# shiv-vignesh/T5-Resnet-VQA

Hardware: AMD Instinct MI355X
Metric: question-image pairs/sec, ResNet50+T5-base+SGA train step, 1/2/4/8 MI355X (higher is better)
Workload: dtype bf16; 1 GPU; ResNet50 + t5-base + 3xSGA train step (BASELINE configs[1]; configs[2] at N=8); model=resnet50+t5-base+3xSGA, global_batch=64, per_gpu_batch=64, seq_len=32, image_size=224, answers=170, parallelism=dp1, world_size=1, graph=True, resnet_pipelined=True

## Files before the change

include/vqa_hip.h:

```cpp
#ifndef VQA_HIP_H
#define VQA_HIP_H

#include <hip/hip_runtime.h>

#ifdef __cplusplus
extern "C" {
#endif

#define VQA_ABI_VERSION 22
#define VQA_OK 0
#define VQA_ERR_INVALID 1000

int vqa_abi_version(void);
const char* vqa_last_error(void);

typedef struct vqa_dropout {
  float p;
  unsigned site;
  const unsigned* rng;
} vqa_dropout;

int vqa_rng_advance(unsigned* rng, hipStream_t stream);
int vqa_dropout_mask(const vqa_dropout* d, float* out, long long n, hipStream_t stream);

// ... 232 lines not shown

int vqa_eval_rows(const vqa_eval_desc* d, hipStream_t stream);

#define VQA_MAX_GROUPS 8
#define VQA_ST_STEP 0
#define VQA_ST_GRAD_NORM 1
#define VQA_ST_CLIP_COEF 2
#define VQA_ST_LR_SCALE 3
#define VQA_ST_BC1 4
#define VQA_ST_BC2_SQRT 5
#define VQA_ST_PENDING 8

typedef struct vqa_adamw_desc {
  float* param; const float* grad;
  float* exp_avg; float* exp_avg_sq; float* max_exp_avg_sq;
  void* param16;
  long long n;
  int ngroups;
  long long group_end[VQA_MAX_GROUPS];
  float group_lr[VQA_MAX_GROUPS];
  float beta1, beta2, eps, weight_decay, grad_scale;
  const float* state;
} vqa_adamw_desc;

int vqa_grad_sqnorm(const float* g, long long n, double* ws, int parts, hipStream_t stream);
int vqa_optim_finalize(const double* ws, int parts, float grad_scale, float max_norm, int warmup, int total,
                       float beta1, float beta2, float* state, hipStream_t stream);
#define VQA_SQNORM_FINAL_COUNTER_WORDS 2112
int vqa_grad_sqnorm_final(const float* g0, long long n0, const float* g1, long long n1, double* ws, int parts,
                          int fin_parts, const int* mark, long long lead, int cols, unsigned* counter,
                          float grad_scale, float max_norm, int warmup, int total, float beta1, float beta2,
                          float* state, hipStream_t stream);
int vqa_adamw_amsgrad(const vqa_adamw_desc* d, hipStream_t stream);
int vqa_embed_mark(const long long* ids, int n, int rows, int* mark, const float* state, hipStream_t stream);
int vqa_adamw_rows(const vqa_adamw_desc* d, const int* mark, int rows, int cols, int touched, int warmup, int total,
                   hipStream_t stream);

#ifdef __cplusplus
}
#endif
#endif
```

t5-resnet-vqa_amd/csrc/adamw.h:

```cpp
#pragma once
#include "common.h"

namespace {

struct AdamArgs {
  float* p; const float* g; float* m; float* v; float* vm; bf16_t* p16;
  long n4;
  int ngroups; long gend4[VQA_MAX_GROUPS]; float glr[VQA_MAX_GROUPS];
  float b1, b2, eps, wd, gscale;
  const float* st;
};

inline int adam_args(const vqa_adamw_desc* d, AdamArgs& A) {
  VQA_REQUIRE(d && d->param && d->grad && d->exp_avg && d->exp_avg_sq && d->max_exp_avg_sq && d->state,
              "vqa_adamw: null argument");
  VQA_REQUIRE(d->n > 0 && d->n % 4 == 0 && d->ngroups >= 1 && d->ngroups <= VQA_MAX_GROUPS, "vqa_adamw: bad sizes");
  VQA_REQUIRE((((uintptr_t)d->param | (uintptr_t)d->grad | (uintptr_t)d->exp_avg | (uintptr_t)d->exp_avg_sq |
                (uintptr_t)d->max_exp_avg_sq) & 15) == 0 && ((uintptr_t)d->param16 & 7) == 0,
              "vqa_adamw: the fp32 streams must be 16-byte aligned, param16 8-byte aligned");
  A.p = d->param; A.g = d->grad; A.m = d->exp_avg; A.v = d->exp_avg_sq; A.vm = d->max_exp_avg_sq;
  A.p16 = (bf16_t*)d->param16;
  A.n4 = d->n / 4;
  A.ngroups = d->ngroups;
  for (int i = 0; i < VQA_MAX_GROUPS; ++i) {
    VQA_REQUIRE(i >= d->ngroups || d->group_end[i] % 4 == 0, "vqa_adamw: group ends must be multiples of 4");
    A.gend4[i] = i < d->ngroups ? d->group_end[i] / 4 : A.n4;
    A.glr[i] = i < d->ngroups ? d->group_lr[i] : 0.f;
  }
  A.b1 = d->beta1; A.b2 = d->beta2; A.eps = d->eps; A.wd = d->weight_decay; A.gscale = d->grad_scale;
  A.st = d->state;
  return VQA_OK;
}

__device__ __forceinline__ void adamw_update4_with(const AdamArgs& A, long i, f32x4_t& p, const f32x4_t g4,
                                                   f32x4_t& m, f32x4_t& v, f32x4_t& vm, const float coef,
                                                   const float lam, const float bc1, const float bc2s) {
#pragma clang fp contract(off)
  const float gmul = A.gscale * coef;
  const float omb1 = 1.f - A.b1, omb2 = 1.f - A.b2;
  int gi = 0;
#pragma unroll
  for (int k = 0; k < VQA_MAX_GROUPS - 1; ++k) gi += (k < A.ngroups - 1 && i >= A.gend4[k]) ? 1 : 0;
  const float lr = A.glr[gi] * lam;
  const float decay = 1.f - lr * A.wd, step_size = lr / bc1;
#pragma unroll
  for (int j = 0; j < 4; ++j) {
    const float gr = g4[j] * gmul;
    p[j] *= decay;
    m[j] = m[j] + omb1 * (gr - m[j]);
    v[j] = v[j] * A.b2 + omb2 * gr * gr;
    vm[j] = fmaxf(vm[j], v[j]);
    const float denom = sqrtf(vm[j]) / bc2s + A.eps;
    p[j] = p[j] - step_size * (m[j] / denom);
  }
}

__device__ __forceinline__ void adamw_update4(const AdamArgs& A, long i, f32x4_t& p, const f32x4_t g4, f32x4_t& m,
                                              f32x4_t& v, f32x4_t& vm) {
  adamw_update4_with(A, i, p, g4, m, v, vm, A.st[VQA_ST_CLIP_COEF], A.st[VQA_ST_LR_SCALE], A.st[VQA_ST_BC1],
                     A.st[VQA_ST_BC2_SQRT]);
}

}
```

t5-resnet-vqa_amd/csrc/optim.hip:

```cpp
#include "adamw.h"

namespace {

__device__ __forceinline__ double sq_term(const float4 v) {
  return (double)v.x * v.x + (double)v.y * v.y + (double)v.z * v.z + (double)v.w * v.w;
}

__device__ __forceinline__ double sq_range(const float* __restrict__ g, long n4, int bid, int nblk) {
  const float4* g4 = reinterpret_cast<const float4*>(g);
  const long st = (long)nblk * 256;
  double s = 0.0;
  long i = (long)bid * 256 + threadIdx.x;
  for (; i + 3 * st < n4; i += 4 * st) {
    float4 v[4];
#pragma unroll
    for (int u = 0; u < 4; ++u) v[u] = g4[i + u * st];
#pragma unroll
    for (int u = 0; u < 4; ++u) s += sq_term(v[u]);
  }
  for (; i < n4; i += st) s += sq_term(g4[i]);
  return s;
}

__device__ __forceinline__ double sq_range_rows(const float* __restrict__ g, long n4, int bid, int nblk,
// ... 118 lines not shown
  s = sq_block_sum(s, red);
  int* flag = reinterpret_cast<int*>(red + 8);
  if (threadIdx.x == 0) {
    __hip_atomic_store((gu64*)(A.ws + (A.fin - 2 * K) + b), (unsigned long long)__double_as_longlong(s),
                       __ATOMIC_RELAXED, __HIP_MEMORY_SCOPE_AGENT);
    asm volatile("s_waitcnt vmcnt(0)" ::: "memory");
    const int nb = 2 * K, grp = b % SQ_NSUB;
    const unsigned members = (unsigned)((nb - grp + SQ_NSUB - 1) / SQ_NSUB);
    const unsigned groups = (unsigned)(nb < SQ_NSUB ? nb : SQ_NSUB);
    gu32* sub = (gu32*)(A.cnt + (1 + grp) * SQ_CNT_STRIDE);
    int last = 0;
    if (__hip_atomic_fetch_add(sub, 1u, __ATOMIC_RELAXED, __HIP_MEMORY_SCOPE_AGENT) == members - 1) {
      __hip_atomic_store(sub, 0u, __ATOMIC_RELAXED, __HIP_MEMORY_SCOPE_AGENT);
      last = __hip_atomic_fetch_add((gu32*)A.cnt, 1u, __ATOMIC_RELAXED, __HIP_MEMORY_SCOPE_AGENT) == groups - 1;
      if (last) __hip_atomic_store((gu32*)A.cnt, 0u, __ATOMIC_RELAXED, __HIP_MEMORY_SCOPE_AGENT);
    }
    *flag = last;
  }
  __syncthreads();
  if (!*flag) return;
  __syncthreads();
  __builtin_amdgcn_fence(__ATOMIC_ACQUIRE, "wavefront");
  finalize_body<true>(A.ws, A.fin, A.grad_scale, A.max_norm, A.warmup, A.total, A.beta1, A.beta2, A.st, red);
}

__global__ __launch_bounds__(256) void embed_mark_kernel(const long long* __restrict__ ids, int n, int rows,
                                                         int* __restrict__ mark, const float* __restrict__ st) {
  const int i = blockIdx.x * 256 + threadIdx.x;
  if (i >= n) return;
  const long long id = ids[i];
  if (id >= 0 && id < rows) mark[id] = (int)st[VQA_ST_STEP];
}

template <int MODE>
__global__ __launch_bounds__(192) void adamw_rows_kernel(AdamArgs A, const int* __restrict__ mark, int rows, int d4,
                                                         int warmup, int total) {
  const int step = (int)A.st[VQA_ST_STEP];
  float coef, lam, bc1, bc2s;
  if (MODE == 0) {
    coef = 1.f;
    schedule_at((double)A.st[VQA_ST_STEP], warmup, total, A.b1, A.b2, lam, bc1, bc2s);
  } else {
    if (A.st[VQA_ST_PENDING] == 0.f) return;
    coef = A.st[VQA_ST_CLIP_COEF];
    lam = A.st[VQA_ST_LR_SCALE];
    bc1 = A.st[VQA_ST_BC1];
    bc2s = A.st[VQA_ST_BC2_SQRT];
  }
  for (int row = blockIdx.x; row < rows; row += gridDim.x) {
  const bool touched = mark[row] == (MODE == 0 ? step : step - 1);
  if (MODE == 0 ? touched : !touched) continue;
  for (int c = threadIdx.x; c < d4; c += 192) {
    const long i = (long)row * d4 + c;
    f32x4_t p = __builtin_nontemporal_load(reinterpret_cast<const f32x4_t*>(A.p) + i);
    f32x4_t g4 = {0.f, 0.f, 0.f, 0.f};
    if (MODE == 1) g4 = __builtin_nontemporal_load(reinterpret_cast<const f32x4_t*>(A.g) + i);
    f32x4_t m = __builtin_nontemporal_load(reinterpret_cast<const f32x4_t*>(A.m) + i);
    f32x4_t v = __builtin_nontemporal_load(reinterpret_cast<const f32x4_t*>(A.v) + i);
    f32x4_t vm = __builtin_nontemporal_load(reinterpret_cast<const f32x4_t*>(A.vm) + i);
    adamw_update4_with(A, i, p, g4, m, v, vm, coef, lam, bc1, bc2s);
    __builtin_nontemporal_store(p, reinterpret_cast<f32x4_t*>(A.p) + i);
    __builtin_nontemporal_store(m, reinterpret_cast<f32x4_t*>(A.m) + i);
    __builtin_nontemporal_store(v, reinterpret_cast<f32x4_t*>(A.v) + i);
    __builtin_nontemporal_store(vm, reinterpret_cast<f32x4_t*>(A.vm) + i);
    if (A.p16) {
      uint2 u;
      u.x = (uint32_t)f2bf(p[0]) | ((uint32_t)f2bf(p[1]) << 16);
      u.y = (uint32_t)f2bf(p[2]) | ((uint32_t)f2bf(p[3]) << 16);
      reinterpret_cast<uint2*>(A.p16)[i] = u;
    }
  }
  }
}

__global__ __launch_bounds__(256) void adamw_kernel(AdamArgs A) {
  const long i = (long)blockIdx.x * 256 + threadIdx.x;
  if (i >= A.n4 || A.st[VQA_ST_PENDING] == 0.f) return;
  f32x4_t p = __builtin_nontemporal_load(reinterpret_cast<const f32x4_t*>(A.p) + i);
  const f32x4_t g4 = __builtin_nontemporal_load(reinterpret_cast<const f32x4_t*>(A.g) + i);
  f32x4_t m = __builtin_nontemporal_load(reinterpret_cast<const f32x4_t*>(A.m) + i);
  f32x4_t v = __builtin_nontemporal_load(reinterpret_cast<const f32x4_t*>(A.v) + i);
  f32x4_t vm = __builtin_nontemporal_load(reinterpret_cast<const f32x4_t*>(A.vm) + i);
  adamw_update4(A, i, p, g4, m, v, vm);
  __builtin_nontemporal_store(p, reinterpret_cast<f32x4_t*>(A.p) + i);
  __builtin_nontemporal_store(m, reinterpret_cast<f32x4_t*>(A.m) + i);
  __builtin_nontemporal_store(v, reinterpret_cast<f32x4_t*>(A.v) + i);
  __builtin_nontemporal_store(vm, reinterpret_cast<f32x4_t*>(A.vm) + i);
  if (A.p16) {
    uint2 u;
    u.x = (uint32_t)f2bf(p[0]) | ((uint32_t)f2bf(p[1]) << 16);
    u.y = (uint32_t)f2bf(p[2]) | ((uint32_t)f2bf(p[3]) << 16);
    reinterpret_cast<uint2*>(A.p16)[i] = u;
  }
}

int grid_for(long n4) {
  long b = (n4 + 255) / 256;
  return (int)(b < 4096 ? b : 4096);
}

}

extern "C" int vqa_grad_sqnorm(const float* g, long long n, double* ws, int parts, hipStream_t s) {
  VQA_REQUIRE(g && ws && n % 4 == 0 && parts > 0 && ((uintptr_t)g & 15) == 0,
              "vqa_grad_sqnorm: bad arguments (n %% 4 == 0, g 16-byte aligned)");
  hipLaunchKernelGGL(sqnorm_kernel, dim3(parts), dim3(256), 0, s, g, (long)(n / 4), ws);
  return vqa::check_launch("vqa_grad_sqnorm");
// ... 18 lines not shown
                        (n1 - lead) % cols == 0 && n1 / 4 < (1ll << 31)),
              "vqa_grad_sqnorm_final: range 1 must be `lead` floats then whole rows of `cols` (both %% 4 == 0)");
  SqFinalArgs A;
  A.g0 = g0; A.n4_0 = (long)(n0 / 4); A.g1 = g1; A.n4_1 = (long)(n1 / 4);
  A.ws = ws; A.parts = parts; A.fin = fin_parts;
  A.mark = mark; A.lead4 = (long)(lead / 4); A.d4 = mark ? (unsigned)(cols / 4) : 1u;
  A.cnt = counter;
  A.grad_scale = grad_scale; A.max_norm = max_norm; A.warmup = warmup; A.total = total;
  A.beta1 = beta1; A.beta2 = beta2; A.st = state;
  hipLaunchKernelGGL(sqnorm_final_kernel, dim3(2 * parts), dim3(256), 0, s, A);
  return vqa::check_launch("vqa_grad_sqnorm_final");
}

extern "C" int vqa_adamw_amsgrad(const vqa_adamw_desc* d, hipStream_t s) {
  AdamArgs A;
  if (int rc = adam_args(d, A)) return rc;
  hipLaunchKernelGGL(adamw_kernel, dim3(vqa::cdiv(A.n4, 256)), dim3(256), 0, s, A);
  return vqa::check_launch("vqa_adamw_amsgrad");
}

extern "C" int vqa_embed_mark(const long long* ids, int n, int rows, int* mark, const float* state, hipStream_t s) {
  VQA_REQUIRE(ids && mark && state && n > 0 && rows > 0, "vqa_embed_mark: bad arguments");
  hipLaunchKernelGGL(embed_mark_kernel, dim3(vqa::cdiv(n, 256)), dim3(256), 0, s, ids, n, rows, mark, state);
  return vqa::check_launch("vqa_embed_mark");
}

extern "C" int vqa_adamw_rows(const vqa_adamw_desc* d, const int* mark, int rows, int cols, int touched, int warmup,
                              int total, hipStream_t s) {
  AdamArgs A;
  if (int rc = adam_args(d, A)) return rc;
  VQA_REQUIRE(mark && rows > 0 && cols > 0 && cols % 4 == 0 && (long long)rows * cols == d->n,
              "vqa_adamw_rows: rows x cols must be the descriptor's n (cols %% 4 == 0)");
  const int grid = touched > 1 && touched < rows ? touched : rows;
  if (touched == 1)
    hipLaunchKernelGGL(adamw_rows_kernel<1>, dim3(rows), dim3(192), 0, s, A, mark, rows, cols / 4, warmup, total);
  else
    hipLaunchKernelGGL(adamw_rows_kernel<0>, dim3(grid), dim3(192), 0, s, A, mark, rows, cols / 4, warmup, total);
  return vqa::check_launch("vqa_adamw_rows");
}
```

t5-resnet-vqa_amd/dp.py:

```python
from __future__ import annotations

import os

import numpy as np
import torch

from . import lib as L
from . import ops
from . import synthetic as S
from .engine_base import _after, no_gc_capture


DP_T5_DW_GROUPS = (4, 4, 3, 1)


def dp_t5_dw_groups(layers=12):
    if layers == 12:
        return DP_T5_DW_GROUPS
    g = [layers // 3, layers // 3, layers // 4]
    return tuple(g + [layers - sum(g)])


def plan_buckets(ready_marks, end, min_bytes=24 << 20):
    out, start = [], 0
# ... 251 lines not shown
            full, mine = e.G32[a:a + N * c], e.G32[a + r * c:a + (r + 1) * c]
            if _staged(full, self.group) or dist.get_backend(self.group) == "gloo":
                h = full.cpu()
                dist.all_reduce(h, group=self.group)
                mine.copy_(h[r * c:(r + 1) * c])
                works.append(_Done())
            else:
                out = self.RS_OUT[self.rs_off[bk_index]:self.rs_off[bk_index] + c]
                if COMM_ON_STREAM:
                    dist.reduce_scatter_tensor(out, full, group=self.group, async_op=False)
                    mine.copy_(out)
                    works.append(_OnStream())
                else:
                    works.append(_Then(dist.reduce_scatter_tensor(out, full, group=self.group, async_op=True),
                                       lambda out=out, mine=mine: mine.copy_(out)))
        if b > a + N * c:
            works += allreduce_buckets(e.G32, [(None, a + N * c, b)], self.group)
        return [_All(works)]

    def _sharded_optimizer(self):
        import torch.distributed as dist
        e = self.eng
        s = L.stream_handle()
        self.WS_SQN.zero_()
        for c in self.sq_calls:
            c(s)
        if _staged(self.WS_SQN, self.group):
            h = self.WS_SQN.cpu()
            dist.all_reduce(h, group=self.group)
            self.WS_SQN.copy_(h)
        else:
            dist.all_reduce(self.WS_SQN, group=self.group)
        self.finalize_call(s)
        for c in self.adam_calls:
            c(s)
        e.clear_pending(s)
        N, r = self.world, self.rank
        for a, c, b in self.shards:
            if c == 0:
                continue
            for t in (e.P32, e.P16):
                full, mine = t[a:a + N * c], t[a + r * c:a + (r + 1) * c]
                if _staged(full, self.group):
                    parts = [torch.empty(c, dtype=t.dtype) for _ in range(N)]
                    dist.all_gather(parts, mine.cpu(), group=self.group)
                    full.copy_(torch.cat(parts))
                else:
                    dist.all_gather_into_tensor(full, mine.clone(), group=self.group)
        if e.fp8 and not e.defer_opt:
            self._run(e.quant_all)

    def sync_optimizer_state(self):
        import torch.distributed as dist
        if not self.shard:
            return
        e = self.eng
        N, r = self.world, self.rank
        for a, c, b in self.shards:
            if c == 0:
                continue
            for t in (e.M, e.V, e.VMAX):
                full, mine = t[a:a + N * c], t[a + r * c:a + (r + 1) * c]
                if _staged(full, self.group):
                    parts = [torch.empty(c, dtype=t.dtype) for _ in range(N)]
                    dist.all_gather(parts, mine.cpu(), group=self.group)
                    full.copy_(torch.cat(parts))
# ... 93 lines not shown
                    for k in st["final"]:
                        works[k] = exchange(k, self.buckets[k])
                        mark_done(k, works[k])
                else:
                    ks = st["final"]
                    assert ks == list(range(ks[0], ks[-1] + 1))
                    ws = allreduce_buckets(e.G32, [(None, self.buckets[ks[0]][1], self.buckets[ks[-1]][2])], self.group)
                    for k in ks:
                        works[k] = ws if k == ks[-1] else []
                        mark_done(k, ws)
                    if j == self._sq0_stage and (COMM_ON_STREAM or _staged(e.G32, self.group)):
                        self._sq0_call(L.stream_handle(comm))
        if tm is not None:
            tm["wait"] = (torch.cuda.Event(enable_timing=True), torch.cuda.Event(enable_timing=True))
            tm["wait"][0].record(main)
        for key, ws in works.items():
            for w in ws:
                w.wait()
        _after(main, comm)
        if tm is not None:
            tm["wait"][1].record(main)
        self._play("finish", self.finish_calls)
        return tm

    def _play(self, name, calls):
        if self.graphs is not None:
            self.graphs[name].replay()
        else:
            self._run(calls)

    def capture(self):
        e = self.eng
        e.flush_optimizer()
        e.ROWTOT.fill_(float(e.B * self.world))
        s = torch.cuda.Stream(e.dev)
        s.wait_stream(torch.cuda.current_stream(e.dev))
        saved_rng = e.RNG.clone()
        with torch.cuda.stream(s):
            e._run(e.fwd_calls)
            e.backward()
        torch.cuda.current_stream(e.dev).wait_stream(s)
        torch.cuda.synchronize(e.dev)
        e.RNG.copy_(saved_rng)
        with no_gc_capture():
            self.graphs = self._capture_all(s)

    def _capture_all(self, s):
        e = self.eng
        gs = {}

        def cap(name, fn):
            g = torch.cuda.CUDAGraph()
            with torch.cuda.graph(g, stream=s):
                fn()
            gs[name] = g
        cap("fwd", self._fwd)
        for j, st in enumerate(self.stages):
            cap(f"stage{j}", lambda st=st: self._run_stage(st))
        cap("finish", lambda: self._run(self.finish_calls))
        return gs

    def _fwd(self):
        e = self.eng
        main = torch.cuda.current_stream(e.dev)
        if self._res_a:
            _after(e._rstream, main)
            with torch.cuda.stream(e._rstream):
                self._run(self._res_a)
        e.run_forward_streams()
        if self._res_a:
            _after(main, e._rstream)

    def _exchange_step_start(self):
        e = self.eng
        main = torch.cuda.current_stream(e.dev)
        e.count_call(L.stream_handle(main))
        _after(self._comm, main)
        with torch.cuda.stream(self._comm):
            ws = allreduce_buckets(e.ROWTOT, [(None, 0, 1)], self.group)
            return ws + gather_tensor(e.IDS, self.GIDS, self.group)

    def step(self):
        e = self.eng
        rows = self._exchange_step_start()
        if e.pipeline:
            e.copy_f4(L.stream_handle(torch.cuda.current_stream(e.dev)))
        if self.graphs is not None:
            self.graphs["fwd"].replay()
        else:
            self._fwd()
        for w in rows:
            w.wait()
        _after(torch.cuda.current_stream(e.dev), self._comm)
        tev = self._backward_exchange()
        if self.shard:
            self._sharded_optimizer()
        if self.timing:
            self._ev.append(tev)

    def timing_report(self):
        torch.cuda.synchronize()
        if not self._ev:
            return None
        e = self.eng
        stage_of = {k: j for j, st in enumerate(self.stages) for k in st["final"]}
        stage_of["rows"] = self.rows_stage

        def mean(f):
            return round(float(np.mean([f(t) for t in self._ev])), 1)
        lag = {k: mean(lambda t, k=k: t["stage"][stage_of[k]].elapsed_time(t["done"][k]) * 1e3) for k in stage_of}
        return {"world_size": self.world, "steps": len(self._ev), "stages": self.stage_plan(),
                "embedding_rows_gather": {"bytes": int(self.world * e.T * (e.D * 4 + 8)),
                                          "done_us_after_stage": lag["rows"]},
                "buckets": [{"start": int(a), "stop": int(b), "bytes": int(4 * (b - a)), "stage": stage_of[k],
                             "done_us_after_stage": lag[k]} for k, (_, a, b) in enumerate(self.buckets)],
                "exposed_wait_us_total": mean(lambda t: t["wait"][0].elapsed_time(t["wait"][1]) * 1e3)}
# ... 1 lines not shown
```

t5-resnet-vqa_amd/engine.py:

```python
from __future__ import annotations

import ctypes
import os

import numpy as np
import torch

from . import lib as L
from . import ops
from . import synthetic as S
from .engine_base import (BF16, F32, I64, IGNORE_INDEX, SITE_EMBED, SITE_FINAL, EngineBase, _after,
                          _check_attn_path, _h2d, _Seq, batch_rows, load_rows, load_rows_multi, no_gc_capture,
                          t5_site)
from .layout import ParamLayout, fold_bn, t5_bucket_map
from .sga_stack import SGAGrads, SGAStack, sga_site
from .t5_stack import T5Grads, T5Stack


def stem_s2d_weight(wf):
    co, kh, kw, ci = wf.shape
    w8 = np.zeros((co, 8, 8, ci), np.float32)
    w8[:, :kh, :kw] = wf
    w = w8.reshape(co, 4, 2, 4, 2, ci).transpose(0, 1, 3, 2, 4, 5).reshape(co, 4, 4, 4 * ci)
    return np.concatenate([w, np.zeros((co, 4, 4, 16 - 4 * ci), np.float32)], 3)


class VQAEngine(EngineBase):
    def __init__(self, state_dict, vision="resnet50", batch=64, seq_len=32, image_size=224, device="cuda:0",
                 warmup=10, total=100, num_blocks=3, answer_spaces=170, grad_scale=1.0, max_norm=1.0,
                 betas=(0.9, 0.999), eps=1e-8, weight_decay=0.1, dropout=0.1, seed=0, pipeline=False,
                 t5_dw_group=None, defer_optimizer=True, dw_stream=None, sga_dw_batch=True, pair_bwd=True,
                 language_model="t5-base", fp8=False, sga_attn_group=True, fuse_norm=None):
        super().__init__(device, dropout, seed, warmup, total, max_norm, betas, eps, weight_decay, grad_scale)
        self.fuse_norm = (os.environ.get("VQA_FUSE_NORM", "0") == "1") if fuse_norm is None else bool(fuse_norm)
        self.fuse_norm_kept = []
        self.pipeline = bool(pipeline)
        self.res_order, self.res_head = "first", 4
        self._res_feed = None
        self._rstream_handle = None
        self._rstream_plain = None
        self.EMB_MARK = None
        self.SQ_CNT = None
        self.heat_call = None
        self._fpn_plan = None
        self.vision, self.B, self.L, self.H = vision, batch, seq_len, image_size
        assert image_size % 2 == 0, "the space-to-depth stem needs an even image size"
        self.NB, self.A = num_blocks, answer_spaces
        self.dims = dm = S.lm_dims(language_model)
        self.D, self.nl, self.h5, self.dkv, self.dff = dm.d_model, dm.t5_layers, dm.t5_heads, dm.t5_dkv, dm.t5_dff
        self.sga_heads, self.sga_dh = dm.sga_heads, dm.sga_dhead
        assert self.h5 * self.dkv == self.D and self.sga_heads * self.sga_dh == self.D
        self.fp8 = bool(fp8)
        if not 1 <= answer_spaces <= 1024:
            raise ValueError(f"answer_spaces={answer_spaces}: the fused answer head supports 1..1024 answers")
        if not 1 <= seq_len <= 64:
            raise ValueError(f"seq_len={seq_len}: the attention / pooler kernels support 1..64 question tokens")
        self.pair_bwd = bool(pair_bwd)
        if t5_dw_group is None:
            t5_dw_group = (3 * self.nl // 4, self.nl - 3 * self.nl // 4)
        if isinstance(t5_dw_group, (list, tuple)):
            self.t5_dw_groups = [int(x) for x in t5_dw_group]
        elif int(t5_dw_group) == 1:
            self.t5_dw_groups = None
        else:
            G = int(t5_dw_group)
            assert G > 1, "t5_dw_group: a group size >= 1 or a sequence of sizes"
            self.t5_dw_groups = [G] * (self.nl // G) + [self.nl % G] * (self.nl % G > 0)
        assert self.t5_dw_groups is None or (sum(self.t5_dw_groups) == self.nl and min(self.t5_dw_groups) >= 1)
        self.sga_dw_batch = bool(sga_dw_batch)
        self.sga_attn_group = bool(sga_attn_group)
        self.defer_opt = bool(defer_optimizer)
        self.dw_stream = True if dw_stream is None else bool(dw_stream)
        self.T = batch * seq_len
        self.rows = batch
# ... 406 lines not shown
            if quant[name]:
                c = _Seq([c] + quant[name])
            if name == "embed":
                self.adam_embed = c
            else:
                self.adam_segs.append((name, c))
        lst = []
        self._call(lst, "vqa_zero", ops.addr(self.opt_state, L.ST_PENDING), 16, extra=[self.opt_state])
        self.clear_pending = lst[0]
        if not self.defer_opt:
            o.append(self.adam_full)
            o += self.quant_all
        elif self.adam_embed is not None:
            o.append(self.adam_embed)
        self.embed_split = self.defer_opt
        self.tail_calls = o[2:]
        self.emb_pre = []
        if self.embed_split:
            emb = lay["t5.embed"]
            assert emb.offset + emb.numel == n and self.adam_embed is o[-1]
            if self.EMB_MARK is None:
                self.EMB_MARK = torch.full((S.T5_VOCAB,), -1, dtype=torch.int32, device=self.dev)
            lo = emb.offset
            self._emb_desc = dt = self._adam_range_desc(lo, n)
            keep = self._adam_keep() + (self.EMB_MARK,)
            rows_call = lambda touched: ops.Call("vqa_adamw_rows", ctypes.byref(dt), self.EMB_MARK.data_ptr(),
                                                 S.T5_VOCAB, self.D, touched, int(self.warmup), int(self.total),
                                                 desc=dt, keep=keep)
            self.emb_pre = [ops.Call("vqa_embed_mark", self.IDS.data_ptr(), self.T, S.T5_VOCAB,
                                     self.EMB_MARK.data_ptr(), self.opt_state.data_ptr(),
                                     keep=(self.IDS, self.EMB_MARK, self.opt_state)),
                            rows_call(256)]
            self.tail_calls = o[2:-1] + [self.adam_range_call(lay["t5.relbias"].offset, lo), rows_call(1)]
        self.tail_calls_unfused = self.tail_calls
        T = self.T
        self.fused_tail = self.embed_split and T <= 16384
        self.emb_sort_call = self.emb_scatter_call = None
        if self.fused_tail:
            if self.SQ_CNT is None:
                self.SQ_CNT = torch.zeros(L.SQNORM_FINAL_COUNTER_WORDS, dtype=torch.int32,
                                          device=self.dev)
            emb = lay["t5.embed"]
            lead = emb.offset - e0
            assert lead >= 0 and lead % 4 == 0 and emb.numel == S.T5_VOCAB * self.D and self.D % 4 == 0
            fin = ops.Call("vqa_grad_sqnorm_final", ops.addr(self.G32, a), e0 - a, ops.addr(self.G32, e0), n - e0,
                           self.WS_SQ.data_ptr(), K, 3 * K, self.EMB_MARK.data_ptr(), lead, self.D,
                           self.SQ_CNT.data_ptr(), float(self.grad_scale), float(self.max_norm), int(self.warmup),
                           int(self.total), float(self.betas[0]), float(self.betas[1]), self.opt_state.data_ptr(),
                           keep=(self.G32[a:], self.WS_SQ, self.EMB_MARK, self.SQ_CNT, self.opt_state))
            assert [c.name for c in self.tail_calls[:2]] == ["vqa_grad_sqnorm", "vqa_optim_finalize"]
            self.tail_calls = [fin] + self.tail_calls[2:]
            ids, dh, dtab, _, _, _, ws = self.emb_call.args
            self.emb_sort_call = ops.Call("vqa_embedding_sort", ids, T, S.T5_VOCAB, ws, keep=(self.IDS, self.WS_EMB))
            self.emb_scatter_call = ops.Call("vqa_embedding_bwd_sorted", dh, dtab, T, self.D, S.T5_VOCAB, ws,
                                             keep=(self.dH32, self.G32, self.WS_EMB))

    def _adam_groups(self):
        ends, lrs = self.lay.group_of_element()
        return ends, [self.group_lr.get(g, lr) for g, lr in zip(self.lay.groups, lrs)]

    def flush_optimizer(self):
        if self.defer_opt:
            self._run([c for _, c in self.adam_segs] + [self.clear_pending])

    def set_grad_scale(self, s):
        self.grad_scale = float(s)
# ... 29 lines not shown
    def prime(self, images):
        assert self.pipeline, "prime() is for pipelined engines"
        ni = batch_rows({"image_tensors": images}, "image_tensors", self.B, self.allow_empty_rows)
        load_rows(self.IMG, images, ni)
        self._img_rows_next = ni
        self._run(self.res_calls)

    def use_global_rows(self, world):
        i = next(k for k, c in enumerate(self.bwd_calls) if c.name == "vqa_head_bwd")
        old = self.bwd_calls[i]
        if self.count_call is not None:
            assert old.args[-1] == float(world), "use_global_rows: already set for another world size"
            return
        new = ops.Call("vqa_head_bwd", *old.args[:-2], ops.addr(self.ROWTOT), float(world),
                       keep=tuple(old.keep) + (self.ROWTOT,))
        new.side = old.side
        self.bwd_calls[i] = new
        self.count_call = ops.Call("vqa_count_targets", ops.addr(self.TGT), self.B, ops.addr(self.ROWTOT),
                                   keep=(self.TGT, self.ROWTOT))
        self.allow_empty_rows = True
        self.graph = None

    def forward(self):
        self.flush_optimizer()
        super().forward()

    def _run_step_streams(self, optimizer=True):
        self.run_forward_streams()
        if optimizer:
            self._backward_and_tail()
        else:
            self.run_backward_streams()

    def _backward_and_tail(self):
        self.run_backward_streams(sq_overlap=True, sorted_scatter=self.fused_tail)
        self._run(self.tail_calls)

    def run_forward_streams(self):
        main = torch.cuda.current_stream(self.dev)
        side = self._side
        f = self.fwd_calls
        p0, p1, p2 = self._fsplit
        self._run(f[:p0])
        _after(side, main)
        vis, txt = f[p0:p1], f[p1:p2]
        if self.defer_opt:
            self._forward_branches_deferred(main, side, vis, txt)
        else:
            self._forward_branches(main, side, vis, txt)
        self._run(f[p2:])

    def _forward_branches(self, main, side, vis, txt):
        hm, hs = L.stream_handle(main), L.stream_handle(side)
        j = 0
        for i, c in enumerate(vis):
            c(hm)
            upto = (i + 1) * len(txt) // len(vis)
            while j < upto:
                txt[j](hs)
                j += 1
        for c in txt[j:]:
            c(hs)
        _after(main, side)

    def _t5_waits(self, i):
        w = [f"t5.{i}"]
        if self.fuse_norm and i + 1 < self.nl:
# ... 160 lines not shown
            g.replay()
        with torch.cuda.stream(self._rstream):
            self._run(self.res_calls)
        _after(main, self._rstream)

    def _step_pipelined(self):
        main = torch.cuda.current_stream(self.dev)
        if self.res_external:
            self.run_forward_streams()
            self._backward_and_tail()
            return
        if not (torch.cuda.is_current_stream_capturing() and self.res_order == "root"):
            self.copy_f4(L.stream_handle(main))
        _after(self._rstream, main)

        last = self.res_order == "last"
        inter = self.res_order == "interleave"
        if inter:
            self._res_feed = [list(self.res_calls), L.stream_handle(self._rstream)]
        elif not last:
            with torch.cuda.stream(self._rstream):
                self._run(self.res_calls)
        self.run_forward_streams()
        if inter:
            assert not self._res_feed[0], "every ResNet call issued"
            self._res_feed = None
        self._backward_and_tail()
        if last:
            with torch.cuda.stream(self._rstream):
                self._run(self.res_calls)
        _after(main, self._rstream)

    def train_step(self):
        if self.graph is not None and self.res_external:
            self._res_external_step()
            return
        if self.graph is not None and self.pipeline and self.res_order == "root":
            self.copy_f4(L.stream_handle(torch.cuda.current_stream(self.dev)))
        if self.graph is not None:
            for g in self.graph:
                if callable(g):
                    g()
                else:
                    g.replay()
            return
        if self.pipeline:
            assert self.allreduce is None, "pipelined DP steps go through dp.DataParallelStep"
            self._step_pipelined()
            return
        self.forward()
        self.backward()
        if self.allreduce is not None:
            self.allreduce(self.G32)
        self.optimizer_step()

    def capture(self, warm=True, keep_graph=False):
        self._keep_graph = bool(keep_graph)
        self.flush_optimizer()
        s = torch.cuda.Stream(self.dev)
        s.wait_stream(torch.cuda.current_stream(self.dev))
        saved, saved_rng = self.opt_state.clone(), self.RNG.clone()
        with torch.cuda.stream(s):
            if warm:
                self._run(self.fwd_calls)
                self.backward()
        torch.cuda.current_stream(self.dev).wait_stream(s)
        torch.cuda.synchronize(self.dev)
        with no_gc_capture():
            parts = self._capture_parts(s)
        self.opt_state.copy_(saved)
        self.RNG.copy_(saved_rng)
        for g in parts:
            if self._keep_graph and not callable(g):
                g.instantiate()
        self.graph = parts

    def _capture_parts(self, s):
        if self.allreduce is None:
            g = self._new_graph()
            with torch.cuda.graph(g, stream=s):
                if self.pipeline:
                    self._step_pipelined()
                else:
                    self._run_step_streams()
            parts = [g]
        else:
            g1, g2 = self._new_graph(), self._new_graph()
            with torch.cuda.graph(g1, stream=s):
                self.forward()
                self.backward()
            with torch.cuda.graph(g2, stream=s):
                self.optimizer_step()
            ar = self.allreduce
            parts = [g1, lambda: ar(self.G32), g2]
        return parts

    def _eval_setup(self, rollout):
        if self.pipeline:
            raise ValueError("pipelined engines take their images a step early; evaluation has no next batch: "
                             "build the engine with pipeline=False to evaluate")
        super()._eval_setup(rollout)

    def _eval_heat_setup(self, heatmap):
        if heatmap:
            self._plan_heat()

    def _run_eval_streams(self):
        main = torch.cuda.current_stream(self.dev)
        side = self._side
        f = self.fwd_calls
# ... 67 lines not shown
```

t5-resnet-vqa_amd/lib.py:

```python
from __future__ import annotations

import ctypes
import os
import re

import torch

PKG_DIR = os.path.dirname(os.path.abspath(__file__))
LIB_PATH = os.path.join(PKG_DIR, "lib", "libvqa_hip.so")
HEADER = os.path.join(os.path.dirname(PKG_DIR), "include", "vqa_hip.h")

c_void_p, c_int, c_float, c_ll = ctypes.c_void_p, ctypes.c_int, ctypes.c_float, ctypes.c_longlong


class ConvGeom(ctypes.Structure):
    _fields_ = [(n, c_int) for n in ("n", "h", "w", "c", "oh", "ow", "kh", "kw", "stride", "pad")]


class Dropout(ctypes.Structure):
    _fields_ = [("p", c_float), ("site", ctypes.c_uint), ("rng", c_void_p)]


class GemmDesc(ctypes.Structure):
    _fields_ = [
# ... 67 lines not shown
                           f"{[int(r[0]) for r in rows]}")
    return {int(r[0]): tuple(map(int, r[1:7])) + (frozenset(re.findall(r"VQA_TILE_(\w+)", r[7])),) for r in rows}


def _flagged(flag):
    return tuple(c for c, t in _TILE_TABLE.items() if flag in t[6])


_TILE_TABLE = gemm_tile_table()
GEMM_TILES = {c: t[:3] for c, t in _TILE_TABLE.items()}
GEMM_WAVES = {c: t[3:5] for c, t in _TILE_TABLE.items()}
GEMM_PATCH_ONLY = _flagged("PATCH")
GEMM_KC_B_ONLY = _flagged("KC_B")
GEMM_K64_ONLY = _flagged("K1")
GEMM_FP8 = _flagged("FP8")
GEMM_NORM = _flagged("NORM")
GEMM_PAIR = _flagged("PAIR")
GEMM_BK128 = tuple(c for c, t in _TILE_TABLE.items() if t[5] == 128)
GEMM_PLAIN_ONLY = tuple(sorted(GEMM_BK128 + GEMM_K64_ONLY))
GEMM_NO_SPLITK = tuple(sorted(GEMM_PLAIN_ONLY + GEMM_PATCH_ONLY))
NORM_LAYER, NORM_RMS = 1, 2


def gemm_config_fits(cfg, d):
    im2col = bool(d.a_conv or d.b_conv)
    return not ((cfg in GEMM_PATCH_ONLY) != (d.a_conv == 2) or (d.norm and cfg not in GEMM_NORM)
                or (d.fp8 and cfg not in GEMM_FP8) or (cfg in GEMM_KC_B_ONLY and d.b_trans)
                or (cfg in GEMM_PLAIN_ONLY and im2col) or (cfg in GEMM_K64_ONLY and d.k > 64))

ATTN_MFMA, ATTN_LONG, ATTN_VALU = 0, 1, 2
MAX_GROUPS = 8
ST_STEP, ST_GRAD_NORM, ST_CLIP_COEF, ST_LR_SCALE, ST_BC1, ST_BC2_SQRT = range(6)
ST_PENDING, ST_FLOATS = 8, 16


class AdamWDesc(ctypes.Structure):
    _fields_ = [
        ("param", c_void_p), ("grad", c_void_p), ("exp_avg", c_void_p), ("exp_avg_sq", c_void_p),
        ("max_exp_avg_sq", c_void_p), ("param16", c_void_p), ("n", c_ll), ("ngroups", c_int),
        ("group_end", c_ll * MAX_GROUPS), ("group_lr", c_float * MAX_GROUPS),
        ("beta1", c_float), ("beta2", c_float), ("eps", c_float), ("weight_decay", c_float),
        ("grad_scale", c_float), ("state", c_void_p),
    ]


class EvalDesc(ctypes.Structure):
    _fields_ = [
        ("logp", c_void_p), ("targets", c_void_p), ("nll", c_void_p), ("loss", c_void_p), ("similarity", c_void_p),
        ("batch", c_int), ("answers", c_int), ("k", c_int),
        ("topk_idx", c_void_p), ("topk_logp", c_void_p), ("acc", c_void_p),
        ("pred_log", c_void_p), ("tgt_log", c_void_p), ("capacity", c_ll),
    ]


EVAL_MAX_K = 16
EVAL_ACC_INTS = ("steps", "rows", "top1", "topk", "cursor")
EVAL_ACC_F64 = ("loss_sum", "nll_sum", "sim_sum")

_lib = None


def header_symbols():
    txt = open(HEADER).read()
    return sorted(set(re.findall(r"^\s*(?:int|long long|const char\*)\s+(vqa_\w+)\s*\(", txt, re.M)))


def abi_version():
    return int(re.search(r"#define VQA_ABI_VERSION (\d+)", open(HEADER).read()).group(1))


def load():
    global _lib
    if _lib is not None:
        return _lib
    if not os.path.exists(LIB_PATH):
        raise RuntimeError(f"libvqa_hip.so not built at {LIB_PATH}: run `python __graft_entry__.py` "
                           "(make -C t5-resnet-vqa_amd/csrc)")
    lib = ctypes.CDLL(LIB_PATH)
    missing = [s for s in header_symbols() if not hasattr(lib, s)]
    if missing:
        raise RuntimeError(f"libvqa_hip.so lacks exported symbols {missing}")
    lib.vqa_last_error.restype = ctypes.c_char_p
    if lib.vqa_abi_version() != abi_version():
        raise RuntimeError(f"libvqa_hip.so ABI {lib.vqa_abi_version()} != header ABI {abi_version()}: rebuild it")
    lib.vqa_gemm.argtypes = [ctypes.POINTER(GemmDesc), c_void_p]
    lib.vqa_gemm_select.argtypes = [ctypes.POINTER(GemmDesc)]
    lib.vqa_gemm_workspace_bytes.argtypes = [ctypes.POINTER(GemmDesc)]
    lib.vqa_gemm_workspace_bytes.restype = c_ll
    lib.vqa_gemm_pair.argtypes = [ctypes.POINTER(GemmDesc), ctypes.POINTER(GemmDesc), c_void_p]
    lib.vqa_attn_fwd.argtypes = [ctypes.POINTER(AttnDesc), c_void_p]
    lib.vqa_attn_bwd.argtypes = [ctypes.POINTER(AttnDesc), c_void_p]
    lib.vqa_attn_path.argtypes = [ctypes.POINTER(AttnDesc), c_int]
    lib.vqa_attn_probs.argtypes = [ctypes.POINTER(AttnDesc), c_void_p]
    lib.vqa_attn_headmean.argtypes = [ctypes.POINTER(AttnDesc), c_void_p, c_ll, c_void_p]
    lib.vqa_adamw_amsgrad.argtypes = [ctypes.POINTER(AdamWDesc), c_void_p]
    lib.vqa_eval_rows.argtypes = [ctypes.POINTER(EvalDesc), c_void_p]
    lib.vqa_adamw_rows.argtypes = [ctypes.POINTER(AdamWDesc), c_void_p, c_int, c_int, c_int, c_int, c_int, c_void_p]
    for name in ("vqa_norm_bwd_workspace_floats", "vqa_colsum_workspace_floats"):
        getattr(lib, name).argtypes = [c_int, c_int]
    lib.vqa_head_workspace_floats.argtypes = [c_int] * 4
    lib.vqa_norm_bwd_parts.argtypes = [c_int]
    lib.vqa_colsum_parts.argtypes = [c_int]
    for name, argtypes in _SIGS.items():
        fn = getattr(lib, name)
        fn.argtypes = argtypes
        fn.restype = c_int
    _lib = lib
    return lib


_SIGS: dict = {}


def register(name, *argtypes):
    _SIGS[name] = list(argtypes) + [c_void_p]


P = c_void_p
register("vqa_rmsnorm_fwd", P, P, P, P, P, c_int, c_int, c_float, P)
register("vqa_rmsnorm_bwd", P, P, P, P, P, P, P, P, c_float, P, c_int, c_int, P, P, P)
register("vqa_layernorm_fwd", P, P, P, P, P, P, P, c_int, c_int, c_float)
register("vqa_layernorm_bwd", P, P, P, P, P, P, P, P, P, P, P, c_int, c_int, P, P)
register("vqa_rng_advance", P)
register("vqa_dropout_mask", P, P, c_ll)
register("vqa_colsum_partials", P, c_int, c_ll, c_int, P, c_float)
register("vqa_image_to_nhwc8", P, P, c_int, c_int, c_int)
register("vqa_image_to_s2d16", P, P, c_int, c_int, c_int)
register("vqa_resize_linear_u8", P, P, c_int, c_int, c_int, P)
register("vqa_resize_pil_bilinear_u8", P, P, c_int, c_int, c_int, c_int, c_int, P, P, P, c_ll, P)
register("vqa_maxpool3x3s2_nhwc", P, P, c_int, c_int, c_int, c_int, c_int, c_int)
# ... 68 lines not shown
```

Before: 9891 pairs/s.

## Skip moment traffic for cold embedding rows in untouched-row AdamW

Adds a scan kernel that marks T5 embedding rows whose AdamW moments are all zero as cold, so the untouched-row AdamW pass can skip loading and storing m, v and max_v for those rows. It only writes back moments when they become nonzero. The untouched-row kernel is also restructured to handle eight rows per block iteration, which increases memory-level parallelism. The scan runs outside graph capture when state is stale, and a drop call resets cold marks before the optimizer. This adds host-side state tracking and a risk of stale marks if the invalidation paths miss a case.

Result: no change. 9884 pairs/s (-0.1%).

```diff
diff --git a/include/vqa_hip.h b/include/vqa_hip.h
--- a/include/vqa_hip.h
+++ b/include/vqa_hip.h
@@ -288,6 +288,8 @@
                           float grad_scale, float max_norm, int warmup, int total, float beta1, float beta2,
                           float* state, hipStream_t stream);
 int vqa_adamw_amsgrad(const vqa_adamw_desc* d, hipStream_t stream);
+#define VQA_EMB_COLD (-2)
+int vqa_embed_cold_scan(const vqa_adamw_desc* d, int* mark, int rows, int cols, hipStream_t stream);
 int vqa_embed_mark(const long long* ids, int n, int rows, int* mark, const float* state, hipStream_t stream);
 int vqa_adamw_rows(const vqa_adamw_desc* d, const int* mark, int rows, int cols, int touched, int warmup, int total,
                    hipStream_t stream);
diff --git a/t5-resnet-vqa_amd/csrc/adamw.h b/t5-resnet-vqa_amd/csrc/adamw.h
--- a/t5-resnet-vqa_amd/csrc/adamw.h
+++ b/t5-resnet-vqa_amd/csrc/adamw.h
@@ -32,16 +32,20 @@
   return VQA_OK;
 }
 
-__device__ __forceinline__ void adamw_update4_with(const AdamArgs& A, long i, f32x4_t& p, const f32x4_t g4,
-                                                   f32x4_t& m, f32x4_t& v, f32x4_t& vm, const float coef,
-                                                   const float lam, const float bc1, const float bc2s) {
+__device__ __forceinline__ float adamw_group_lr(const AdamArgs& A, long i) {
+  int gi = 0;
+#pragma unroll
+  for (int k = 0; k < VQA_MAX_GROUPS - 1; ++k) gi += (k < A.ngroups - 1 && i >= A.gend4[k]) ? 1 : 0;
+  return A.glr[gi];
+}
+
+__device__ __forceinline__ void adamw_update4_lr(const AdamArgs& A, const float glr, f32x4_t& p, const f32x4_t g4,
+                                                 f32x4_t& m, f32x4_t& v, f32x4_t& vm, const float coef,
+                                                 const float lam, const float bc1, const float bc2s) {
 #pragma clang fp contract(off)
   const float gmul = A.gscale * coef;
   const float omb1 = 1.f - A.b1, omb2 = 1.f - A.b2;
-  int gi = 0;
-#pragma unroll
-  for (int k = 0; k < VQA_MAX_GROUPS - 1; ++k) gi += (k < A.ngroups - 1 && i >= A.gend4[k]) ? 1 : 0;
-  const float lr = A.glr[gi] * lam;
+  const float lr = glr * lam;
   const float decay = 1.f - lr * A.wd, step_size = lr / bc1;
 #pragma unroll
   for (int j = 0; j < 4; ++j) {
@@ -55,6 +59,12 @@
   }
 }
 
+__device__ __forceinline__ void adamw_update4_with(const AdamArgs& A, long i, f32x4_t& p, const f32x4_t g4,
+                                                   f32x4_t& m, f32x4_t& v, f32x4_t& vm, const float coef,
+                                                   const float lam, const float bc1, const float bc2s) {
+  adamw_update4_lr(A, adamw_group_lr(A, i), p, g4, m, v, vm, coef, lam, bc1, bc2s);
+}
+
 __device__ __forceinline__ void adamw_update4(const AdamArgs& A, long i, f32x4_t& p, const f32x4_t g4, f32x4_t& m,
                                               f32x4_t& v, f32x4_t& vm) {
   adamw_update4_with(A, i, p, g4, m, v, vm, A.st[VQA_ST_CLIP_COEF], A.st[VQA_ST_LR_SCALE], A.st[VQA_ST_BC1],
diff --git a/t5-resnet-vqa_amd/csrc/optim.hip b/t5-resnet-vqa_amd/csrc/optim.hip
--- a/t5-resnet-vqa_amd/csrc/optim.hip
+++ b/t5-resnet-vqa_amd/csrc/optim.hip
@@ -174,14 +174,90 @@
   if (id >= 0 && id < rows) mark[id] = (int)st[VQA_ST_STEP];
 }
 
+__device__ __forceinline__ void store_p_p16(const AdamArgs& A, long i, const f32x4_t p) {
+  __builtin_nontemporal_store(p, reinterpret_cast<f32x4_t*>(A.p) + i);
+  if (A.p16) {
+    uint2 u;
+    u.x = (uint32_t)f2bf(p[0]) | ((uint32_t)f2bf(p[1]) << 16);
+    u.y = (uint32_t)f2bf(p[2]) | ((uint32_t)f2bf(p[3]) << 16);
+    reinterpret_cast<uint2*>(A.p16)[i] = u;
+  }
+}
+
+__device__ __forceinline__ unsigned or_bits(const f32x4_t x) {
+  return __float_as_uint(x[0]) | __float_as_uint(x[1]) | __float_as_uint(x[2]) | __float_as_uint(x[3]);
+}
+
+constexpr int EMB_ROWS_R = 8;
+
+__device__ __forceinline__ void adamw_rows_untouched(const AdamArgs& A, int* mark, int rows, int d4, int step,
+                                                     float lam, float bc1, float bc2s) {
+  constexpr int R = EMB_ROWS_R;
+  const f32x4_t zero4 = {0.f, 0.f, 0.f, 0.f};
+  for (long row0 = blockIdx.x; row0 < rows; row0 += (long)R * gridDim.x) {
+    int mv[R], mk[R];
+#pragma unroll
+    for (int u = 0; u < R; ++u) {
+      const long r = row0 + (long)u * gridDim.x;
+      mv[u] = mark[r < rows ? r : rows - 1];
+    }
+#pragma unroll
+    for (int u = 0; u < R; ++u) mk[u] = __builtin_amdgcn_readfirstlane(mv[u]);
+#pragma unroll
+    for (int u = 0; u < R; ++u) mk[u] = row0 + (long)u * gridDim.x < rows ? mk[u] : step;
+    for (int c = threadIdx.x; c < d4; c += 192) {
+      float glr[R];
+#pragma unroll
+      for (int u = 0; u < R; ++u) glr[u] = adamw_group_lr(A, (row0 + (long)u * gridDim.x) * d4 + c);
+      f32x4_t p[R], m[R], v[R], vm[R];
+#pragma unroll
+      for (int u = 0; u < R; ++u) {
+        const long i = (row0 + (long)u * gridDim.x) * d4 + c;
+        p[u] = m[u] = v[u] = vm[u] = zero4;
+        if (mk[u] != step) p[u] = __builtin_nontemporal_load(reinterpret_cast<const f32x4_t*>(A.p) + i);
+        if (mk[u] != step && mk[u] != VQA_EMB_COLD) {
+          m[u] = __builtin_nontemporal_load(reinterpret_cast<const f32x4_t*>(A.m) + i);
+          v[u] = __builtin_nontemporal_load(reinterpret_cast<const f32x4_t*>(A.v) + i);
+          vm[u] = __builtin_nontemporal_load(reinterpret_cast<const f32x4_t*>(A.vm) + i);
+        }
+      }
+#pragma unroll
+      for (int u = 0; u < R; ++u)
+        adamw_update4_lr(A, glr[u], p[u], zero4, m[u], v[u], vm[u], 1.f, lam, bc1, bc2s);
+#pragma unroll
+      for (int u = 0; u < R; ++u) {
+        if (mk[u] == step) continue;
+        const long r = row0 + (long)u * gridDim.x;
+        const long i = r * d4 + c;
+        store_p_p16(A, i, p[u]);
+        bool moments = true;
+        if (mk[u] == VQA_EMB_COLD) {
+          bool inf_nan = false;
+#pragma unroll
+          for (int j = 0; j < 4; ++j) inf_nan |= (__float_as_uint(p[u][j]) & 0x7f800000u) == 0x7f800000u;
+          moments = (or_bits(m[u]) | or_bits(v[u]) | or_bits(vm[u])) != 0u || inf_nan;
+          if (moments) mark[r] = -1;
+        }
+        if (moments) {
+          __builtin_nontemporal_store(m[u], reinterpret_cast<f32x4_t*>(A.m) + i);
+          __builtin_nontemporal_store(v[u], reinterpret_cast<f32x4_t*>(A.v) + i);
+          __builtin_nontemporal_store(vm[u], reinterpret_cast<f32x4_t*>(A.vm) + i);
+        }
+      }
+    }
+  }
+}
+
 template <int MODE>
-__global__ __launch_bounds__(192) void adamw_rows_kernel(AdamArgs A, const int* __restrict__ mark, int rows, int d4,
+__global__ __launch_bounds__(192) void adamw_rows_kernel(AdamArgs A, int* mark, int rows, int d4,
                                                          int warmup, int total) {
   const int step = (int)A.st[VQA_ST_STEP];
   float coef, lam, bc1, bc2s;
   if (MODE == 0) {
     coef = 1.f;
     schedule_at((double)A.st[VQA_ST_STEP], warmup, total, A.b1, A.b2, lam, bc1, bc2s);
+    adamw_rows_untouched(A, mark, rows, d4, step, lam, bc1, bc2s);
+    return;
   } else {
     if (A.st[VQA_ST_PENDING] == 0.f) return;
     coef = A.st[VQA_ST_CLIP_COEF];
@@ -215,6 +291,32 @@
   }
 }
 
+__global__ __launch_bounds__(256) void embed_cold_scan_kernel(AdamArgs A, int* __restrict__ mark, int rows, int d4) {
+  const int step = (int)A.st[VQA_ST_STEP];
+  for (int row = blockIdx.x; row < rows; row += gridDim.x) {
+    const int mk = mark[row];
+    if (mk == step) continue;
+    unsigned bits = 0u;
+    for (int c = threadIdx.x; c < d4; c += 256) {
+      const long i = (long)row * d4 + c;
+      const f32x4_t m = reinterpret_cast<const f32x4_t*>(A.m)[i];
+      const f32x4_t v = reinterpret_cast<const f32x4_t*>(A.v)[i];
+      const f32x4_t vm = reinterpret_cast<const f32x4_t*>(A.vm)[i];
+      bits |= or_bits(m) | or_bits(v) | or_bits(vm);
+    }
+    const int warm = __syncthreads_or(bits != 0u);
+    if (threadIdx.x == 0) {
+      if (!warm) mark[row] = VQA_EMB_COLD;
+      else if (mk == VQA_EMB_COLD) mark[row] = -1;
+    }
+  }
+}
+
+__global__ __launch_bounds__(256) void embed_cold_drop_kernel(int* __restrict__ mark, int rows) {
+  const int i = blockIdx.x * 256 + threadIdx.x;
+  if (i < rows && mark[i] == VQA_EMB_COLD) mark[i] = -1;
+}
+
 __global__ __launch_bounds__(256) void adamw_kernel(AdamArgs A) {
   const long i = (long)blockIdx.x * 256 + threadIdx.x;
   if (i >= A.n4 || A.st[VQA_ST_PENDING] == 0.f) return;
@@ -299,9 +401,23 @@
   VQA_REQUIRE(mark && rows > 0 && cols > 0 && cols % 4 == 0 && (long long)rows * cols == d->n,
               "vqa_adamw_rows: rows x cols must be the descriptor's n (cols %% 4 == 0)");
   const int grid = touched > 1 && touched < rows ? touched : rows;
+  int* mk = const_cast<int*>(mark);
   if (touched == 1)
-    hipLaunchKernelGGL(adamw_rows_kernel<1>, dim3(rows), dim3(192), 0, s, A, mark, rows, cols / 4, warmup, total);
+    hipLaunchKernelGGL(adamw_rows_kernel<1>, dim3(rows), dim3(192), 0, s, A, mk, rows, cols / 4, warmup, total);
   else
-    hipLaunchKernelGGL(adamw_rows_kernel<0>, dim3(grid), dim3(192), 0, s, A, mark, rows, cols / 4, warmup, total);
+    hipLaunchKernelGGL(adamw_rows_kernel<0>, dim3(grid), dim3(192), 0, s, A, mk, rows, cols / 4, warmup, total);
   return vqa::check_launch("vqa_adamw_rows");
 }
+
+extern "C" int vqa_embed_cold_scan(const vqa_adamw_desc* d, int* mark, int rows, int cols, hipStream_t s) {
+  VQA_REQUIRE(mark && rows > 0 && cols > 0 && cols % 4 == 0, "vqa_embed_cold_scan: bad arguments (cols %% 4 == 0)");
+  if (!d) {
+    hipLaunchKernelGGL(embed_cold_drop_kernel, dim3(vqa::cdiv(rows, 256)), dim3(256), 0, s, mark, rows);
+    return vqa::check_launch("vqa_embed_cold_scan");
+  }
+  AdamArgs A;
+  if (int rc = adam_args(d, A)) return rc;
+  VQA_REQUIRE((long long)rows * cols == d->n, "vqa_embed_cold_scan: rows x cols must be the descriptor's n");
+  hipLaunchKernelGGL(embed_cold_scan_kernel, dim3(rows < 2048 ? rows : 2048), dim3(256), 0, s, A, mark, rows, cols / 4);
+  return vqa::check_launch("vqa_embed_cold_scan");
+}
diff --git a/t5-resnet-vqa_amd/dp.py b/t5-resnet-vqa_amd/dp.py
--- a/t5-resnet-vqa_amd/dp.py
+++ b/t5-resnet-vqa_amd/dp.py
@@ -307,6 +307,7 @@
         else:
             dist.all_reduce(self.WS_SQN, group=self.group)
         self.finalize_call(s)
+        e._cold_drop()
         for c in self.adam_calls:
             c(s)
         e.clear_pending(s)
@@ -466,6 +467,8 @@
     def capture(self):
         e = self.eng
         e.flush_optimizer()
+        if self.emb_pre:
+            e._cold_scan()
         e.ROWTOT.fill_(float(e.B * self.world))
         s = torch.cuda.Stream(e.dev)
         s.wait_stream(torch.cuda.current_stream(e.dev))
@@ -516,6 +519,8 @@
 
     def step(self):
         e = self.eng
+        if self.emb_pre:
+            e._cold_scan()
         rows = self._exchange_step_start()
         if e.pipeline:
             e.copy_f4(L.stream_handle(torch.cuda.current_stream(e.dev)))
diff --git a/t5-resnet-vqa_amd/engine.py b/t5-resnet-vqa_amd/engine.py
--- a/t5-resnet-vqa_amd/engine.py
+++ b/t5-resnet-vqa_amd/engine.py
@@ -30,7 +30,7 @@
                  warmup=10, total=100, num_blocks=3, answer_spaces=170, grad_scale=1.0, max_norm=1.0,
                  betas=(0.9, 0.999), eps=1e-8, weight_decay=0.1, dropout=0.1, seed=0, pipeline=False,
                  t5_dw_group=None, defer_optimizer=True, dw_stream=None, sga_dw_batch=True, pair_bwd=True,
-                 language_model="t5-base", fp8=False, sga_attn_group=True, fuse_norm=None):
+                 language_model="t5-base", fp8=False, sga_attn_group=True, fuse_norm=None, embed_cold=True):
         super().__init__(device, dropout, seed, warmup, total, max_norm, betas, eps, weight_decay, grad_scale)
         self.fuse_norm = (os.environ.get("VQA_FUSE_NORM", "0") == "1") if fuse_norm is None else bool(fuse_norm)
         self.fuse_norm_kept = []
@@ -40,6 +40,10 @@
         self._rstream_handle = None
         self._rstream_plain = None
         self.EMB_MARK = None
+        self.embed_cold = bool(embed_cold)
+        self._cold_stale = True
+        self._graph_split = False
+        self.cold_scan_call = self.cold_drop_call = None
         self.SQ_CNT = None
         self.heat_call = None
         self._fpn_plan = None
@@ -512,6 +516,12 @@
                                      keep=(self.IDS, self.EMB_MARK, self.opt_state)),
                             rows_call(256)]
             self.tail_calls = o[2:-1] + [self.adam_range_call(lay["t5.relbias"].offset, lo), rows_call(1)]
+            self.cold_scan_call = ops.Call("vqa_embed_cold_scan", ctypes.byref(dt), self.EMB_MARK.data_ptr(),
+                                           S.T5_VOCAB, self.D, desc=dt, keep=keep)
+            self.cold_drop_call = ops.Call("vqa_embed_cold_scan", None, self.EMB_MARK.data_ptr(), S.T5_VOCAB, self.D,
+                                           keep=(self.EMB_MARK,))
+            o.insert(len(o) - 1, self.cold_drop_call)
+            self._cold_stale = True
         self.tail_calls_unfused = self.tail_calls
         T = self.T
         self.fused_tail = self.embed_split and T <= 16384
@@ -607,7 +617,27 @@
         else:
             self.run_backward_streams()
 
+    def _cold_scan(self):
+        if (self.embed_cold and self._cold_stale and self.cold_scan_call is not None
+                and not torch.cuda.is_current_stream_capturing()):
+            self._run([self.cold_scan_call])
+            self._cold_stale = False
+
+    def _cold_drop(self):
+        if self.cold_drop_call is not None:
+            self._run([self.cold_drop_call])
+        self._cold_stale = True
+
+    def optimizer_step(self):
+        self._cold_stale = True
+        super().optimizer_step()
+
+    def load_optimizer_state(self, *a, **kw):
+        self._cold_drop()
+        super().load_optimizer_state(*a, **kw)
+
     def _backward_and_tail(self):
+        self._cold_scan()
         self.run_backward_streams(sq_overlap=True, sorted_scatter=self.fused_tail)
         self._run(self.tail_calls)
 
@@ -834,6 +864,11 @@
         _after(main, self._rstream)
 
     def train_step(self):
+        if self.graph is not None:
+            if self._graph_split:
+                self._cold_scan()
+            else:
+                self._cold_stale = True
         if self.graph is not None and self.res_external:
             self._res_external_step()
             return
@@ -859,6 +894,8 @@
     def capture(self, warm=True, keep_graph=False):
         self._keep_graph = bool(keep_graph)
         self.flush_optimizer()
+        if self.allreduce is None:
+            self._cold_scan()
         s = torch.cuda.Stream(self.dev)
         s.wait_stream(torch.cuda.current_stream(self.dev))
         saved, saved_rng = self.opt_state.clone(), self.RNG.clone()
@@ -878,6 +915,7 @@
         self.graph = parts
 
     def _capture_parts(self, s):
+        self._graph_split = self.allreduce is None
         if self.allreduce is None:
             g = self._new_graph()
             with torch.cuda.graph(g, stream=s):
diff --git a/t5-resnet-vqa_amd/lib.py b/t5-resnet-vqa_amd/lib.py
--- a/t5-resnet-vqa_amd/lib.py
+++ b/t5-resnet-vqa_amd/lib.py
@@ -123,6 +123,7 @@
 MAX_GROUPS = 8
 ST_STEP, ST_GRAD_NORM, ST_CLIP_COEF, ST_LR_SCALE, ST_BC1, ST_BC2_SQRT = range(6)
 ST_PENDING, ST_FLOATS = 8, 16
+EMB_COLD = -2
 
 
 class AdamWDesc(ctypes.Structure):
@@ -187,6 +188,7 @@
     lib.vqa_adamw_amsgrad.argtypes = [ctypes.POINTER(AdamWDesc), c_void_p]
     lib.vqa_eval_rows.argtypes = [ctypes.POINTER(EvalDesc), c_void_p]
     lib.vqa_adamw_rows.argtypes = [ctypes.POINTER(AdamWDesc), c_void_p, c_int, c_int, c_int, c_int, c_int, c_void_p]
+    lib.vqa_embed_cold_scan.argtypes = [ctypes.POINTER(AdamWDesc), c_void_p, c_int, c_int, c_void_p]
     for name in ("vqa_norm_bwd_workspace_floats", "vqa_colsum_workspace_floats"):
         getattr(lib, name).argtypes = [c_int, c_int]
     lib.vqa_head_workspace_floats.argtypes = [c_int] * 4
```
